# kangxiongbin/HyLight

Hardware: AMD Instinct MI355X
Metric: long-read all-vs-all overlaps/sec (higher is better)
Workload: dtype u8/int32

## Files before the change

### hylight_amd/csrc/filter_stage.hip

```cpp
#include "filter_stage.h"

#include <memory>

#include <algorithm>

#include "dev_prims.h"
#include "dev_search.h"
#include "wave_ops.h"

namespace hlmi {

namespace {

constexpr int WINDOW = 1000;
constexpr int QUERY_CAP = 60;
constexpr int WG = 256;

__device__ __forceinline__ uint64_t pair_key(uint32_t a, uint32_t b) {
    return a <= b ? ((uint64_t)a << 32 | b) : ((uint64_t)b << 32 | a);
}

__device__ __forceinline__ bool is_internal(const PafRec &r, int min_o) {
    int64_t ql = r.qlen, qs = r.qs, qe = r.qe, tl = r.tlen, ts = r.ts, te = r.te;
    if (r.flags & PF_REV) {
// ... 262 lines not shown
        size_t j = i;
        while (j > b && row_less(recs[x], recs[grows[j - 1]], ops)) { grows[j] = grows[j - 1]; --j; }
        grows[j] = x;
    }
    bool taken = false;
    for (size_t i = b; i < e; ++i) {
        const PafRec &r = recs[grows[i]];
        bool s1 = false;
        if (r.qid != r.tid) {
            if (long_mode) {
                if (!(r.flags & PF_STAR) && !taken) { s1 = true; taken = true; }
            } else {
                s1 = true;
            }
        }
        sel[i] = s1;
    }
}

constexpr uint32_t NO_PAIR = 0xffffffffu;
__device__ __forceinline__ uint32_t wave_incl_sum_u32(uint32_t v, int lane) {
    (void)lane;
    return wave_prefix_sum_incl_dpp(v);
}

__global__ __launch_bounds__(WG) void snp_count_kernel(const PafRec *recs, const uint32_t *ops, const uint32_t *grows,
                                                        const uint8_t *sel, size_t n, int long_mode, uint32_t *n_ev,
                                                        uint32_t *n_iv, uint32_t *maxv) {
    const int lane = threadIdx.x & 63;
    const size_t wave = (blockIdx.x * (size_t)blockDim.x + threadIdx.x) >> 6;
    const size_t n_waves = ((size_t)gridDim.x * blockDim.x) >> 6;
    uint32_t max_id = 0, max_len = 0;
    for (size_t i = wave; i < n; i += n_waves) {
        uint32_t ne = 0, ni = 0;
        if (sel[i]) {
            const PafRec &r = recs[grows[i]];
            max_id = max(max_id, max(r.qid, r.tid));
            max_len = max(max_len, max(r.qlen, r.tlen));
            const uint32_t *o = ops + r.cig_off;
            for (uint32_t k0 = 0; k0 < r.cig_n; k0 += 64)
                ne += (uint32_t)__popcll(__ballot(k0 + lane < r.cig_n && (o[k0 + lane] & 15u) == OP_X));
            if (long_mode) ne *= 2;
            ni = (r.ts < r.te ? 1u : 0u) + ((long_mode && r.qs < r.qe) ? 1u : 0u);
        }
        if (lane == 0) { n_ev[i] = ne; n_iv[i] = ni; }
    }
    if (lane == 0) {
        if (max_id > __hip_atomic_load(&maxv[0], __ATOMIC_RELAXED, __HIP_MEMORY_SCOPE_AGENT)) atomicMax(&maxv[0], max_id);
        if (max_len > __hip_atomic_load(&maxv[1], __ATOMIC_RELAXED, __HIP_MEMORY_SCOPE_AGENT)) atomicMax(&maxv[1], max_len);
    }
}

__global__ __launch_bounds__(WG) void snp_fill_kernel(const PafRec *recs, const uint32_t *ops, const uint32_t *grows,
                                                       const uint8_t *sel, size_t n, int long_mode, const uint32_t *ev_off,
                                                       const uint32_t *iv_off, const uint32_t *row_pair, int hb, int lb,
                                                       uint64_t *ev_ck, uint32_t *ev_pair,
                                                       uint64_t *iv_sck, uint64_t *iv_eck) {
    auto ck = [&](uint32_t chunk, uint32_t id, uint32_t pos) { return ((uint64_t)chunk << hb | id) << lb | pos; };
    const int lane = threadIdx.x & 63;
    const size_t wave = (blockIdx.x * (size_t)blockDim.x + threadIdx.x) >> 6;
    const size_t n_waves = ((size_t)gridDim.x * blockDim.x) >> 6;
    for (size_t i = wave; i < n; i += n_waves) {
        if (!sel[i]) continue;
        const PafRec r = recs[grows[i]];
        if (lane == 0) {
            uint32_t w = iv_off[i];
            if (r.ts < r.te) { iv_sck[w] = ck(r.chunk, r.tid, r.ts); iv_eck[w] = ck(r.chunk, r.tid, r.te); ++w; }
            if (long_mode && r.qs < r.qe) { iv_sck[w] = ck(r.chunk, r.qid, r.qs); iv_eck[w] = ck(r.chunk, r.qid, r.qe); }
        }
        const uint32_t pg = row_pair[i];
        const bool rev = r.flags & PF_REV;
        uint32_t p1 = rev ? r.qlen - r.qe : r.qs;
        uint32_t p2 = r.ts;
        uint32_t e = ev_off[i];
        const uint32_t *o = ops + r.cig_off;
        for (uint32_t k0 = 0; k0 < r.cig_n; k0 += 64) {
            uint32_t len = 0, code = 0;
            if (k0 + lane < r.cig_n) { const uint32_t op = o[k0 + lane]; len = op >> 4; code = op & 15u; }
            const bool isx = code == OP_X;
            const uint32_t d1 = (code == OP_EQ || code == OP_I || isx) ? len : 0u;
            const uint32_t d2 = (code == OP_EQ || code == OP_D || isx) ? len : 0u;
            const uint32_t s1 = wave_incl_sum_u32(d1, lane), s2 = wave_incl_sum_u32(d2, lane);
            const unsigned long long xm = __ballot(isx);
            if (isx) {
                const uint32_t q1 = p1 + s1, q2 = p2 + s2;
                uint32_t at = e + (uint32_t)__popcll(xm & ((1ull << lane) - 1ull)) * (long_mode ? 2u : 1u);
                if (long_mode) {
                    const uint32_t qp = rev ? r.qlen - q1 + 1 : q1;
                    ev_ck[at] = ck(r.chunk, r.qid, qp); ev_pair[at] = pg; ++at;
                }
                ev_ck[at] = ck(r.chunk, r.tid, q2); ev_pair[at] = pg;
            }
            p1 += (uint32_t)__shfl((int)s1, 63, 64);
            p2 += (uint32_t)__shfl((int)s2, 63, 64);
            e += (uint32_t)__popcll(xm) * (long_mode ? 2u : 1u);
        }
    }
}

__global__ void snp_support_kernel(const uint64_t *ev_ck, const uint32_t *kseg_start, size_t n_kseg, size_t n_ev,
                                   const uint64_t *ivs_ck, const uint64_t *ive_ck, size_t n_iv, int lb, int mc,
                                   uint8_t *ev_supported) {
    size_t s = blockIdx.x * (size_t)blockDim.x + threadIdx.x;
    if (s >= n_kseg) return;
    size_t b = kseg_start[s], e = (s + 1 < n_kseg) ? kseg_start[s + 1] : n_ev;
    int64_t v = (int64_t)(e - b);
    if (v < mc) return;
    const uint64_t key = ev_ck[b];
    const uint64_t read0 = key >> lb << lb;
    const size_t a = lower_bound_u64(ivs_ck, n_iv, read0);
    const uint64_t next_read = read0 + (1ull << lb);
    size_t span = n_iv - a < 4096 ? n_iv - a : 4096;
    if (span == 4096 && ivs_ck[a + span - 1] < next_read) span = n_iv - a;
    const size_t b_ = a + lower_bound_u64(ivs_ck + a, span, next_read);
    const int64_t n_start_lt = (int64_t)lower_bound_u64(ivs_ck + a, b_ - a, key);
    const int64_t n_end_le = (int64_t)lower_bound_u64(ive_ck + a, b_ - a, key + 1);
    int64_t con = n_start_lt - n_end_le;
    if (con - v < mc) return;
    for (size_t i = b; i < e; ++i) ev_supported[i] = 1;
}

__global__ void snp_pair_count_kernel(const uint32_t *ev_pair_sorted, const uint8_t *ev_supported, size_t n_ev,
                                      uint32_t *pair_mut) {
    size_t i = blockIdx.x * (size_t)blockDim.x + threadIdx.x;
    if (i < n_ev && ev_supported[i]) {
        const uint32_t pg = ev_pair_sorted[i];
        if (pg != NO_PAIR) atomicAdd(&pair_mut[pg], 1u);
    }
}

constexpr int PILE_TILE = 15360;
constexpr int PILE_WG_HEAVY = 1024;
constexpr int PILE_LIGHT_ROWS = 16;
constexpr int PILE_EV_SLOTS = 4096;
constexpr uint32_t PILE_MAX_ROWS = 60000;

__global__ void pile_entries_kernel(const PafRec *recs, const uint32_t *grows, const uint8_t *sel, size_t m, int long_mode,
                                    uint64_t *key, uint32_t *val) {
    size_t i = blockIdx.x * (size_t)blockDim.x + threadIdx.x;
    if (i >= m) return;
    uint64_t kt = ~0ull, kq = ~0ull;
    if (sel[i]) {
        const PafRec &r = recs[grows[i]];
        kt = (uint64_t)r.chunk << 32 | r.tid;
        if (long_mode) kq = (uint64_t)r.chunk << 32 | r.qid;
    }
    key[2 * i] = kt; val[2 * i] = (uint32_t)(i << 1);
    key[2 * i + 1] = kq; val[2 * i + 1] = (uint32_t)(i << 1 | 1u);
}
__global__ void pile_entry_rows_kernel(const uint32_t *ent_val, const uint32_t *grows, size_t n, uint32_t *ent_rec) {
    size_t k = blockIdx.x * (size_t)blockDim.x + threadIdx.x;
    if (k < n) ent_rec[k] = grows[ent_val[k] >> 1];
}
__global__ void add_one_u8_kernel(const uint8_t *in, uint8_t *out, size_t n) {
    size_t i = blockIdx.x * (size_t)blockDim.x + threadIdx.x;
    if (i < n) out[i] = in[i] + 1;
}
__global__ void pile_seg_size_kernel(const uint32_t *seg_start, size_t n_seg, size_t n_ent, uint32_t *max_rows) {
    size_t s = blockIdx.x * (size_t)blockDim.x + threadIdx.x;
    if (s >= n_seg) return;
    const uint32_t n = (uint32_t)((s + 1 < n_seg ? seg_start[s + 1] : n_ent) - seg_start[s]);
    if (n > __hip_atomic_load(max_rows, __ATOMIC_RELAXED, __HIP_MEMORY_SCOPE_AGENT)) atomicMax(max_rows, n);
}

template <typename CT> __device__ __forceinline__ void lds_inc(uint32_t *a, uint32_t idx) {
    constexpr uint32_t per = 4 / sizeof(CT);
    atomicAdd(&a[idx / per], 1u << (8 * sizeof(CT) * (idx % per)));
}
template <typename CT> __device__ __forceinline__ uint32_t lds_get(const uint32_t *a, uint32_t idx) { return ((const CT *)a)[idx]; }

__global__ void pile_seg_class_kernel(const uint32_t *seg_start, size_t n_seg, size_t n_ent, int mc, uint8_t *cls) {
    size_t s = blockIdx.x * (size_t)blockDim.x + threadIdx.x;
    if (s >= n_seg) return;
    const uint32_t n = (uint32_t)((s + 1 < n_seg ? seg_start[s + 1] : n_ent) - seg_start[s]);
    cls[s] = (long long)n < 2ll * mc ? 0 : (n <= (uint32_t)PILE_LIGHT_ROWS ? 1 : 2);
}
__global__ __launch_bounds__(WG) void pile_tiny_events_kernel(const PafRec *recs, const uint32_t *ops, const uint32_t *grows,
                                                               const uint32_t *ent_val, const uint32_t *seg_start, const uint32_t *list,
                                                               size_t n_list, size_t n_seg, size_t n_ent, unsigned long long *n_events) {
    const int lane = threadIdx.x & 63;
    const size_t w = (blockIdx.x * (size_t)blockDim.x + threadIdx.x) >> 6;
    if (w >= n_list) return;
    const size_t seg = list[w];
    const size_t b = seg_start[seg], e = seg + 1 < n_seg ? seg_start[seg + 1] : n_ent;
    unsigned long long ev = 0;
    for (size_t k = b; k < e; ++k) {
        const PafRec &r = recs[grows[ent_val[k] >> 1]];
        const uint32_t *o = ops + r.cig_off;
        for (uint32_t k0 = 0; k0 < r.cig_n; k0 += 64)
            ev += (unsigned long long)__popcll(__ballot(k0 + lane < r.cig_n && (o[k0 + lane] & 15u) == OP_X));
    }
    if (lane == 0 && ev) atomicAdd(&n_events[w & (PILE_EV_SLOTS - 1)], ev);
}

template <int PILE_WG, typename CT>
__global__ __launch_bounds__(PILE_WG) __attribute__((amdgpu_waves_per_eu(8, 8))) void snp_pileup_kernel(const PafRec *recs, const uint32_t *ops, const uint32_t *ent_rec,
                                                              const uint32_t *row_pair, const uint64_t *ent_key, const uint32_t *ent_val,
                                                              const uint32_t *seg_start, const uint32_t *list, size_t n_seg, size_t n_ent,
                                                              int long_mode, int mc, uint32_t *pair_mut, unsigned long long *n_events) {
    constexpr uint32_t PER = 4 / sizeof(CT);
    __shared__ uint32_t sA[PILE_TILE / PER], sB[PILE_TILE / PER];
    __shared__ uint32_t s_part[2][PILE_WG / 64];
    const int tid = threadIdx.x, lane = tid & 63, wave = tid >> 6;
    const size_t seg = list[blockIdx.x];
    const size_t b = seg_start[seg], e = seg + 1 < n_seg ? seg_start[seg + 1] : n_ent;
    __shared__ uint32_t s_len;
    if (tid == 0) s_len = 0;
    __syncthreads();
    {
        uint32_t l = 0;
        for (size_t k = b + (size_t)tid; k < e; k += PILE_WG) {
            const uint32_t v = ent_val[k];
            const PafRec &r = recs[ent_rec[k]];
            l = max(l, (v & 1u) ? r.qlen : r.tlen);
        }
        if (l) atomicMax(&s_len, l);
    }
    __syncthreads();
    const uint32_t read_len = s_len;
    auto walk = [&](const PafRec &r, bool qside, auto &&f) {
        const bool rev = r.flags & PF_REV;
        uint32_t p = qside ? (rev ? r.qlen - r.qe : r.qs) : r.ts;
        const uint32_t skip = qside ? OP_D : OP_I;
        const uint32_t *o = ops + r.cig_off;
        for (uint32_t k0 = 0; k0 < r.cig_n; k0 += 256) {
            uint32_t opv[4];
#pragma unroll
            for (int u = 0; u < 4; ++u) { const uint32_t idx = k0 + 64u * u + lane; opv[u] = idx < r.cig_n ? o[idx] : skip; }
#pragma unroll
            for (int u = 0; u < 4; ++u) {
                if (k0 + 64u * u >= r.cig_n) break;
                const uint32_t len = opv[u] >> 4, code = opv[u] & 15u;
                const bool isx = code == OP_X;
                const uint32_t sc = wave_prefix_sum_incl_dpp(code == skip ? 0u : len);
                const uint32_t after = p + sc;
                f(qside && rev ? r.qlen - after + 1 : after, isx);
                p += (uint32_t)__builtin_amdgcn_readlane((int)sc, 63);
            }
        }
    };
    unsigned long long ev = 0;
    for (uint32_t t0 = 0; t0 < read_len + 2; t0 += PILE_TILE) {
        const uint32_t n_pos = min((uint32_t)PILE_TILE, read_len + 2 - t0), n_words = (n_pos + PER - 1) / PER;
        for (uint32_t w = tid; w < n_words; w += PILE_WG) { sA[w] = 0; sB[w] = 0; }
        __syncthreads();
        for (size_t k = b + (size_t)tid; k < e; k += PILE_WG) {
            const uint32_t v = ent_val[k];
            const PafRec &r = recs[ent_rec[k]];
            const uint32_t s0 = (v & 1u) ? r.qs : r.ts, e0 = (v & 1u) ? r.qe : r.te;
            if (s0 < e0) {
                const uint32_t ia = max(s0 + 1, t0) - t0, ib = max(e0, t0) - t0;
                if (ia < n_pos) lds_inc<CT>(sA, ia);
                if (ib < n_pos) lds_inc<CT>(sB, ib);
            }
        }
        __syncthreads();
        {
            const uint32_t per = (n_pos + PILE_WG - 1) / PILE_WG, lo = min(n_pos, (uint32_t)tid * per), hi = min(n_pos, lo + per);
            uint32_t ta = 0, tb = 0;
            for (uint32_t i = lo; i < hi; ++i) { ta += lds_get<CT>(sA, i); tb += lds_get<CT>(sB, i); }
            const uint32_t ia = wave_prefix_sum_incl_dpp(ta), ib = wave_prefix_sum_incl_dpp(tb);
            if (lane == 63) { s_part[0][wave] = ia; s_part[1][wave] = ib; }
            __syncthreads();
            uint32_t oa = ia - ta, ob = ib - tb;
            for (int w = 0; w < wave; ++w) { oa += s_part[0][w]; ob += s_part[1][w]; }
            CT *ca = (CT *)sA, *cb = (CT *)sB;
            for (uint32_t i = lo; i < hi; ++i) {
                oa += ca[i]; ob += cb[i];
                ca[i] = (CT)(oa - ob);
                cb[i] = 0;
            }
        }
        __syncthreads();
        {
            size_t k = b + (size_t)wave;
            uint32_t v = 0;
            PafRec r{};
            if (k < e) { v = ent_val[k]; r = recs[ent_rec[k]]; }
            while (k < e) {
                const size_t kn = k + PILE_WG / 64;
                uint32_t vn = 0;
                PafRec rn{};
                if (kn < e) { vn = ent_val[kn]; rn = recs[ent_rec[kn]]; }
                walk(r, (v & 1u) != 0, [&](uint32_t pos, bool isx) {
                    if (isx && pos >= t0 && pos - t0 < n_pos) lds_inc<CT>(sB, pos - t0);
                    if (t0 == 0) ev += (unsigned long long)__popcll(__ballot(isx));
                });
                k = kn; v = vn; r = rn;
            }
        }
        __syncthreads();
        {
            auto next_live = [&](size_t k) {
                while (k < e && row_pair[ent_val[k] >> 1] == NO_PAIR) k += PILE_WG / 64;
                return k;
            };
            size_t k = next_live(b + (size_t)wave);
            uint32_t v = 0;
            PafRec r{};
            if (k < e) { v = ent_val[k]; r = recs[ent_rec[k]]; }
            while (k < e) {
                const size_t kn = next_live(k + PILE_WG / 64);
                uint32_t vn = 0;
                PafRec rn{};
                if (kn < e) { vn = ent_val[kn]; rn = recs[ent_rec[kn]]; }
                uint32_t hits = 0;
                walk(r, (v & 1u) != 0, [&](uint32_t pos, bool isx) {
                    if (isx && pos >= t0 && pos - t0 < n_pos) {
                        const int cnt = (int)lds_get<CT>(sB, pos - t0), cov = (int)lds_get<CT>(sA, pos - t0);
                        if (cnt >= mc && cov - cnt >= mc) ++hits;
                    }
                });
                hits = wave_incl_sum_u32(hits, lane);
                if (lane == 63 && hits) atomicAdd(&pair_mut[row_pair[v >> 1]], hits);
                k = kn; v = vn; r = rn;
            }
        }
        __syncthreads();
    }
    if (lane == 0 && ev) atomicAdd(&n_events[(blockIdx.x * 16u + (uint32_t)wave) & (PILE_EV_SLOTS - 1)], ev);
}

constexpr int PILE_LIGHT_WG = 512, PILE_LIGHT_IT = 6;
__global__ __launch_bounds__(PILE_LIGHT_WG) void snp_pileup_light_kernel(const PafRec *recs, const uint32_t *ops, const uint32_t *ent_rec,
                                                                          const uint32_t *row_pair, const uint32_t *ent_val,
                                                                          const uint32_t *seg_start, const uint32_t *list, size_t n_seg,
                                                                          size_t n_ent, int mc, uint32_t *pair_mut,
                                                                          unsigned long long *n_events) {
    __shared__ uint32_t sV[PILE_TILE / 4];
    __shared__ uint32_t s_is[PILE_LIGHT_ROWS], s_ie[PILE_LIGHT_ROWS], s_len;
    __shared__ uint32_t s_ev[PILE_LIGHT_ROWS * 64 * PILE_LIGHT_IT], s_nev, s_hits[PILE_LIGHT_ROWS], s_pair[PILE_LIGHT_ROWS];
    const int tid = threadIdx.x, lane = tid & 63, wave = tid >> 6;
    const size_t seg = list[blockIdx.x];
    const size_t b = seg_start[seg], e = seg + 1 < n_seg ? seg_start[seg + 1] : n_ent;
    const int n_rows = (int)(e - b);
    if (tid == 0) s_len = 0;
    if (tid < PILE_LIGHT_ROWS) s_pair[tid] = NO_PAIR;
    __syncthreads();
    uint32_t pos[2][PILE_LIGHT_IT];
    uint32_t xm[2] = {0, 0}, pg[2] = {NO_PAIR, NO_PAIR};
    bool spill[2] = {false, false};
    PafRec rr[2];
    bool side[2] = {false, false};
    unsigned long long ev = 0;
#pragma unroll
    for (int sl = 0; sl < 2; ++sl) {
        const int k = wave + 8 * sl;
        if (k >= n_rows) continue;
        const uint32_t v = ent_val[b + k];
        const PafRec r = recs[ent_rec[b + k]];
        rr[sl] = r; side[sl] = (v & 1u) != 0;
        pg[sl] = row_pair[v >> 1];
        const bool qside = side[sl], rev = r.flags & PF_REV;
        if (lane == 0) {
            const uint32_t s0 = qside ? r.qs : r.ts, e0 = qside ? r.qe : r.te;
            s_is[k] = s0 < e0 ? s0 : 0; s_ie[k] = s0 < e0 ? e0 : 0;
            s_pair[k] = pg[sl];
            atomicMax(&s_len, qside ? r.qlen : r.tlen);
        }
        spill[sl] = r.cig_n > 64u * PILE_LIGHT_IT;
        uint32_t p = qside ? (rev ? r.qlen - r.qe : r.qs) : r.ts;
        const uint32_t skip = qside ? OP_D : OP_I;
        const uint32_t *o = ops + r.cig_off;
        uint32_t opv[PILE_LIGHT_IT];
#pragma unroll
        for (int u = 0; u < PILE_LIGHT_IT; ++u) { const uint32_t idx = 64u * u + lane; opv[u] = idx < r.cig_n ? o[idx] : skip; }
#pragma unroll
        for (int u = 0; u < PILE_LIGHT_IT; ++u) {
            const uint32_t len = opv[u] >> 4, code = opv[u] & 15u;
            const uint32_t sc = wave_prefix_sum_incl_dpp(code == skip ? 0u : len);
            const uint32_t after = p + sc;
            pos[sl][u] = qside && rev ? r.qlen - after + 1 : after;
            if (code == OP_X) xm[sl] |= 1u << u;
            p += (uint32_t)__builtin_amdgcn_readlane((int)sc, 63);
        }
        for (uint32_t k0 = 0; k0 < r.cig_n; k0 += 64)
            ev += (unsigned long long)__popcll(__ballot(k0 + lane < r.cig_n && (k0 < 64u * PILE_LIGHT_IT ? ((xm[sl] >> (k0 >> 6)) & 1u) != 0
                                                                                 : (o[k0 + lane] & 15u) == OP_X)));
    }
    __syncthreads();
    const uint32_t read_len = s_len;
    auto tail = [&](int sl, auto &&f) {
        const PafRec &r = rr[sl];
        const bool qside = side[sl], rev = r.flags & PF_REV;
        const uint32_t skip = qside ? OP_D : OP_I;
        const uint32_t *o = ops + r.cig_off;
        uint32_t p = qside ? (rev ? r.qlen - r.qe : r.qs) : r.ts;
        for (uint32_t k0 = 0; k0 < r.cig_n; k0 += 64) {
            uint32_t len = 0, code = skip;
            if (k0 + lane < r.cig_n) { const uint32_t op = o[k0 + lane]; len = op >> 4; code = op & 15u; }
            const uint32_t sc = wave_prefix_sum_incl_dpp(code == skip ? 0u : len);
            const uint32_t after = p + sc;
            if (k0 >= 64u * PILE_LIGHT_IT) f(qside && rev ? r.qlen - after + 1 : after, code == OP_X);
            p += (uint32_t)__builtin_amdgcn_readlane((int)sc, 63);
        }
    };
    for (uint32_t t0 = 0; t0 < read_len + 2; t0 += PILE_TILE) {
        const uint32_t n_pos = min((uint32_t)PILE_TILE, read_len + 2 - t0);
        for (uint32_t w = tid; w < (n_pos + 3) / 4; w += PILE_LIGHT_WG) sV[w] = 0;
        if (tid < PILE_LIGHT_ROWS) s_hits[tid] = 0;
        if (tid == 0) s_nev = 0;
        __syncthreads();
#pragma unroll
        for (int sl = 0; sl < 2; ++sl) {
            if (wave + 8 * sl >= n_rows) continue;
#pragma unroll
            for (int u = 0; u < PILE_LIGHT_IT; ++u) {
                const bool in = ((xm[sl] >> u) & 1u) && pos[sl][u] >= t0 && pos[sl][u] - t0 < n_pos;
                if (in) lds_inc<uint8_t>(sV, pos[sl][u] - t0);
                if (pg[sl] != NO_PAIR) {
                    const unsigned long long m = __ballot(in);
                    if (m) {
                        uint32_t at = 0;
                        if (lane == 0) at = atomicAdd(&s_nev, (uint32_t)__popcll(m));
                        at = (uint32_t)__builtin_amdgcn_readfirstlane((int)at);
                        if (in) s_ev[at + (uint32_t)__popcll(m & ((1ull << lane) - 1ull))] = (pos[sl][u] - t0) | (uint32_t)(wave + 8 * sl) << 16;
                    }
                }
            }
            if (spill[sl]) tail(sl, [&](uint32_t q, bool isx) { if (isx && q >= t0 && q - t0 < n_pos) lds_inc<uint8_t>(sV, q - t0); });
        }
        __syncthreads();
        auto supported = [&](uint32_t q) {
            const int cnt = (int)lds_get<uint8_t>(sV, q - t0);
            if (cnt < mc) return false;
            int cov = 0;
            for (int i = 0; i < n_rows; ++i) cov += (s_is[i] < q && q < s_ie[i]) ? 1 : 0;
            return cov - cnt >= mc;
        };
        {
            const uint32_t n_ev = s_nev;
            for (uint32_t i = tid; i < n_ev; i += PILE_LIGHT_WG) {
                const uint32_t w = s_ev[i];
                if (supported(t0 + (w & 0xffffu))) atomicAdd(&s_hits[w >> 16], 1u);
            }
        }
#pragma unroll
        for (int sl = 0; sl < 2; ++sl) {
            if (wave + 8 * sl >= n_rows || pg[sl] == NO_PAIR || !spill[sl]) continue;
            uint32_t hits = 0;
            tail(sl, [&](uint32_t q, bool isx) { if (isx && q >= t0 && q - t0 < n_pos && supported(q)) ++hits; });
            hits = wave_prefix_sum_incl_dpp(hits);
            if (lane == 63 && hits) atomicAdd(&s_hits[wave + 8 * sl], hits);
        }
        __syncthreads();
        if (tid < PILE_LIGHT_ROWS && s_hits[tid]) atomicAdd(&pair_mut[s_pair[tid]], s_hits[tid]);
        __syncthreads();
    }
    if (lane == 0 && ev) atomicAdd(&n_events[(blockIdx.x * 16u + (uint32_t)wave) & (PILE_EV_SLOTS - 1)], ev);
}

__global__ void pair_live_kernel(const PafRec *recs, const uint32_t *grows, const uint32_t *seg_start, size_t n_seg,
                                 size_t n_rows, int len_over, int min_o, uint32_t *row_pair) {
    size_t s = blockIdx.x * (size_t)blockDim.x + threadIdx.x;
    if (s >= n_seg) return;
    size_t b = seg_start[s], e = (s + 1 < n_seg) ? seg_start[s + 1] : n_rows;
    bool any = false;
    for (size_t i = b; i < e && !any; ++i) {
        const PafRec &r = recs[grows[i]];
        any = r.qid != r.tid && (int64_t)r.nmatch >= (int64_t)len_over && !is_internal(r, min_o);
    }
    for (size_t i = b; i < e; ++i) row_pair[i] = any ? (uint32_t)s : 0xffffffffu;
}

__global__ void pass2_kernel(const PafRec *recs, const uint32_t *ops, const uint32_t *grows,
                             const uint32_t *seg_start, size_t n_seg, size_t n_rows, const uint32_t *pair_mut,
                             int long_mode, int len_over, double thre, int min_o, uint8_t *keep, uint32_t *xdig) {
    size_t s = blockIdx.x * (size_t)blockDim.x + threadIdx.x;
    if (s >= n_seg) return;
    size_t b = seg_start[s], e = (s + 1 < n_seg) ? seg_start[s + 1] : n_rows;
    const uint32_t mut = pair_mut[s];
    bool done = false;
    for (size_t i = b; i < e; ++i) {
        keep[i] = 0;
        if (done) continue;
        const PafRec &r = recs[grows[i]];
        if (mut > 0) {
            if (!long_mode) continue;
            if ((double)mut / (double)r.nmatch > thre) continue;
        }
        if (r.qid == r.tid) continue;
        if ((int64_t)r.nmatch < (int64_t)len_over) continue;
        if (is_internal(r, min_o)) continue;
        done = true;
        keep[i] = 1;
        uint32_t sum = 0;
        const uint32_t *o = ops + r.cig_off;
        for (uint32_t k = 0; k < r.cig_n; ++k)
            if ((o[k] & 15u) == OP_X) sum += (o[k] >> 4) % 10u;
        xdig[i] = sum;
    }
}

std::vector<uint64_t> make_windows(const std::vector<uint64_t> &chunk_row_start, std::vector<uint32_t> &len) {
    std::vector<uint64_t> start;
    for (size_t c = 0; c + 1 < chunk_row_start.size(); ++c)
        for (uint64_t p = chunk_row_start[c]; p < chunk_row_start[c + 1]; p += WINDOW) {
            start.push_back(p);
            len.push_back((uint32_t)std::min<uint64_t>(WINDOW, chunk_row_start[c + 1] - p));
        }
    return start;
}

}

namespace {
__global__ void chunk_ops_kernel(const PafRec *recs, size_t n, unsigned long long *ops_of_chunk) {
    size_t i = blockIdx.x * (size_t)blockDim.x + threadIdx.x;
    const bool live = i < n;
    const uint32_t c = live ? recs[i].chunk : 0xffffffffu;
    unsigned long long v = live ? recs[i].cig_n : 0;
    const uint32_t c0 = (uint32_t)__shfl((int)c, 0, 64);
    if (__all(!live || c == c0)) {
#pragma unroll
        for (int o = 32; o > 0; o >>= 1) v += __shfl_xor(v, o, 64);
        if ((threadIdx.x & 63) == 0 && v) atomicAdd(&ops_of_chunk[c0], v);
    } else if (live && v) {
        atomicAdd(&ops_of_chunk[c], v);
    }
}
}

std::vector<uint64_t> ops_per_chunk(const PafRec *d_recs, size_t n, uint32_t n_chunk_ids) {
    DBuf<unsigned long long> acc(n_chunk_ids ? n_chunk_ids : 1);
    acc.zero();
    if (n) hipLaunchKernelGGL(chunk_ops_kernel, grid1(n), dim3(WG), 0, stream(), d_recs, n, acc.p);
    HIP_CHECK(hipGetLastError());
    std::vector<unsigned long long> h = acc.download(n_chunk_ids);
    return std::vector<uint64_t>(h.begin(), h.end());
}

std::vector<PafRec> download_rows(const PafRec *d_recs, const std::vector<uint32_t> &idx) {
    std::vector<PafRec> out;
    if (idx.empty()) return out;
    DBuf<uint32_t> d_idx;
    d_idx.upload(idx);
    DBuf<PafRec> tmp(idx.size());
    hipLaunchKernelGGL(gather_rec_kernel, grid1(idx.size()), dim3(WG), 0, stream(), d_recs, d_idx.p, tmp.p, idx.size());
    HIP_CHECK(hipGetLastError());
    return tmp.download(idx.size());
}

void window_filter_device(const PafRec *d_recs, size_t n, const std::vector<uint64_t> &chunk_row_start, int variant,
                          int min_len, double min_iden, int min_o, uint8_t *d_keep) {
    if (!n) return;
    std::vector<uint32_t> wlen;
    std::vector<uint64_t> wstart = make_windows(chunk_row_start, wlen);
    DBuf<uint64_t> d_ws;
    DBuf<uint32_t> d_wl;
    d_ws.upload(wstart);
    d_wl.upload(wlen);
    if (variant == 4)
        hipLaunchKernelGGL(window_filter_kernel<4>, dim3((unsigned)wstart.size()), dim3(WG), 0, stream(), d_recs, d_ws.p,
                           d_wl.p, min_len, min_iden, min_o, d_keep);
    else if (variant == 3)
        hipLaunchKernelGGL(window_filter_kernel<3>, dim3((unsigned)wstart.size()), dim3(WG), 0, stream(), d_recs, d_ws.p,
                           d_wl.p, min_len, min_iden, min_o, d_keep);
    else
        fail(HLMI_EINVAL, "window filter variant must be 3 or 4");
    HIP_CHECK(hipGetLastError());
    sync();
}

void ovlp_inline_device(const PafRec *d_recs, size_t n, int min_len, double min_iden, int o, double r, uint8_t *d_keep,
                        uint32_t *d_first_of) {
    if (!n) return;
    std::vector<uint32_t> wlen;
    std::vector<uint64_t> wstart = make_windows({0, (uint64_t)n}, wlen);
    DBuf<uint64_t> d_ws;
    DBuf<uint32_t> d_wl;
    d_ws.upload(wstart);
    d_wl.upload(wlen);
    hipLaunchKernelGGL(ovlp_inline_kernel, dim3((unsigned)wstart.size()), dim3(WG), 0, stream(), d_recs, d_ws.p, d_wl.p, min_len,
                       min_iden, o, r, d_keep, d_first_of);
    HIP_CHECK(hipGetLastError());
    sync();
}

void filter_stage_device(const PafRec *d_recs, size_t n, const uint32_t *d_ops,
                         const std::vector<uint64_t> &chunk_row_start, const FilterCfg &cfg, FilterOut &out) {
    out = FilterOut();
    if (!n) return;
    const uint32_t n_chunks = std::max<uint32_t>((uint32_t)(chunk_row_start.size() - 1), cfg.chunk_id_bound);
    const int lm = cfg.long_mode ? 1 : 0;

    std::unique_ptr<HostTimer> ht(new HostTimer("filter_v4_select"));
    DBuf<uint8_t> keep1(n);
    { KTimer kt("filter_v4");
    window_filter_device(d_recs, n, chunk_row_start, 4, cfg.v4_min_len, cfg.v4_min_iden, cfg.v4_min_o, keep1.p);
    }
    DBuf<uint32_t> rows(n);
    const size_t m = select_flagged_indices(keep1.p, rows.p, n);
    out.n_after_v4 = m;
    if (!m) return;

    ht.reset(); ht.reset(new HostTimer("filter_pair_groups"));
    DBuf<uint32_t> rchunk(m);
    DBuf<uint64_t> rkey(m);
    hipLaunchKernelGGL(pair_keys_kernel, grid1(m), dim3(WG), 0, stream(), d_recs, rows.p, m, rchunk.p, rkey.p);
    SortedCK g;
    sort_chunk_key(rchunk.p, rkey.p, m, n_chunks, g);
    DBuf<uint32_t> grows(m);
    hipLaunchKernelGGL(gather_u32_kernel, grid1(m), dim3(WG), 0, stream(), rows.p, g.perm.p, grows.p, m);
    DBuf<uint8_t> head(m);
    hipLaunchKernelGGL(head_flags_kernel, grid1(m), dim3(WG), 0, stream(), g.chunk.p, g.key.p, head.p, m);
    DBuf<uint32_t> pseg_start(m);
    const size_t n_pseg = select_flagged_indices(head.p, pseg_start.p, m);
    out.n_pairs = n_pseg;
    DBuf<uint8_t> sel(m);
    hipLaunchKernelGGL(pair_order_select_kernel, grid1(n_pseg), dim3(WG), 0, stream(), d_recs, d_ops, grows.p, pseg_start.p,
                       n_pseg, m, lm, sel.p);

    ht.reset(); ht.reset(new HostTimer("filter_events"));
    DBuf<uint32_t> pair_mut(n_pseg);
    pair_mut.zero();
    bool piled = false;
    if (!hook("HLMI_SNP_SORT")) {
        DBuf<uint64_t> ekey(2 * m);
        DBuf<uint32_t> eval(2 * m);
        hipLaunchKernelGGL(pile_entries_kernel, grid1(m), dim3(WG), 0, stream(), d_recs, grows.p, sel.p, m, lm, ekey.p, eval.p);
        sort_pairs_u64_u32(ekey, eval, 2 * m, 0, 32 + bits_for(n_chunks > 1 ? n_chunks - 1 : 1));
        DBuf<uint32_t> eseg(2 * m);
        size_t n_eseg = select_run_heads_u64(ekey.p, 2 * m, 0, eseg.p);
        size_t n_ent = 2 * m;
        if (n_eseg && download_one(ekey.p + (2 * m - 1)) == ~0ull) { --n_eseg; n_ent = download_one(eseg.p + n_eseg); }
        DBuf<uint32_t> max_rows(1);
        max_rows.zero();
        if (n_eseg) hipLaunchKernelGGL(pile_seg_size_kernel, grid1(n_eseg), dim3(WG), 0, stream(), eseg.p, n_eseg, n_ent, max_rows.p);
        if (!n_eseg || download_one(max_rows.p) <= PILE_MAX_ROWS) {
            DBuf<uint32_t> row_pair(m);
            DBuf<unsigned long long> n_ev_d(PILE_EV_SLOTS);
            n_ev_d.zero();
            hipLaunchKernelGGL(pair_live_kernel, grid1(n_pseg), dim3(WG), 0, stream(), d_recs, grows.p, pseg_start.p, n_pseg, m,
                               cfg.len_over, cfg.min_o, row_pair.p);
            if (n_eseg) {
                DBuf<uint32_t> erec(n_ent);
                hipLaunchKernelGGL(pile_entry_rows_kernel, grid1(n_ent), dim3(WG), 0, stream(), eval.p, grows.p, n_ent, erec.p);
                DBuf<uint8_t> cls(n_eseg);
                hipLaunchKernelGGL(pile_seg_class_kernel, grid1(n_eseg), dim3(WG), 0, stream(), eseg.p, n_eseg, n_ent, cfg.mc, cls.p);
                DBuf<uint32_t> l0(n_eseg), l1(n_eseg), l2(n_eseg), l3(1), cnt4(4);
                DBuf<uint8_t> cls1(n_eseg);
                hipLaunchKernelGGL(add_one_u8_kernel, grid1(n_eseg), dim3(WG), 0, stream(), cls.p, cls1.p, n_eseg);
                select_classes4_async(cls1.p, n_eseg, l0.p, l1.p, l2.p, l3.p, cnt4.p);
                const std::vector<uint32_t> nc = cnt4.download(4);
                if (nc[0]) hipLaunchKernelGGL(pile_tiny_events_kernel, dim3(cdiv(nc[0], (size_t)(WG / 64))), dim3(WG), 0, stream(), d_recs,
                                              d_ops, grows.p, eval.p, eseg.p, l0.p, (size_t)nc[0], n_eseg, n_ent, n_ev_d.p);
                if (nc[1]) {
                    KTimer kt("filter_pileup_light");
                    hipLaunchKernelGGL(snp_pileup_light_kernel, dim3(nc[1]), dim3(PILE_LIGHT_WG), 0, stream(), d_recs, d_ops, erec.p,
                                       row_pair.p, eval.p, eseg.p, l1.p, n_eseg, n_ent, cfg.mc, pair_mut.p, n_ev_d.p);
                }
                if (nc[2]) {
                    KTimer kt("filter_pileup_heavy");
                    hipLaunchKernelGGL((snp_pileup_kernel<PILE_WG_HEAVY, uint16_t>), dim3(nc[2]), dim3(PILE_WG_HEAVY), 0, stream(), d_recs, d_ops, erec.p,
                                       row_pair.p, ekey.p, eval.p, eseg.p, l2.p, n_eseg, n_ent, lm, cfg.mc, pair_mut.p, n_ev_d.p);
                }
            }
            HIP_CHECK(hipGetLastError());
            {
                const std::vector<unsigned long long> evs = n_ev_d.download(PILE_EV_SLOTS);
                unsigned long long tot = 0;
                for (unsigned long long v : evs) tot += v;
                out.n_events = (size_t)tot;
            }
            piled = true;
        }
    }
    if (!piled) {
    DBuf<uint32_t> n_ev(m), n_iv(m), ev_off(m), iv_off(m);
    const dim3 rows_grid((unsigned)std::min<size_t>(cdiv(m ? m : 1, WG / 64), 65536));
    DBuf<uint32_t> maxv(2);
    maxv.zero();
    hipLaunchKernelGGL(snp_count_kernel, rows_grid, dim3(WG), 0, stream(), d_recs, d_ops, grows.p, sel.p, m, lm, n_ev.p,
                       n_iv.p, maxv.p);
    exclusive_scan_u32(n_ev.p, ev_off.p, m);
    exclusive_scan_u32(n_iv.p, iv_off.p, m);
    const size_t E = (size_t)download_one(ev_off.p + (m - 1)) + download_one(n_ev.p + (m - 1));
    const size_t I = (size_t)download_one(iv_off.p + (m - 1)) + download_one(n_iv.p + (m - 1));
    out.n_events = E;
    if (E) {
        const std::vector<uint32_t> mx = maxv.download(2);
        const int cb = bits_for(n_chunks > 1 ? n_chunks - 1 : 1), hb = bits_for(mx[0] ? mx[0] : 1), lb = bits_for((uint64_t)mx[1] + 1);
        if (cb + hb + lb > 64) fail(HLMI_EINVAL, "SNP pile-up key needs %d bits (chunks %d, reads %d, positions %d)", cb + hb + lb, cb, hb, lb);
        DBuf<uint32_t> ev_pair(E);
        DBuf<uint64_t> ev_ck(E), iv_sck(I ? I : 1), iv_eck(I ? I : 1);
    { KTimer kt("filter_event_fill");
        DBuf<uint32_t> row_pair(m);
        hipLaunchKernelGGL(pair_live_kernel, grid1(n_pseg), dim3(WG), 0, stream(), d_recs, grows.p, pseg_start.p, n_pseg, m,
                           cfg.len_over, cfg.min_o, row_pair.p);
        hipLaunchKernelGGL(snp_fill_kernel, rows_grid, dim3(WG), 0, stream(), d_recs, d_ops, grows.p, sel.p, m, lm,
                           ev_off.p, iv_off.p, row_pair.p, hb, lb, ev_ck.p, ev_pair.p, iv_sck.p, iv_eck.p);
    }
    { KTimer kt("filter_event_sort");
        sort_pairs_u64_u32(ev_ck, ev_pair, E, 0, cb + hb + lb);
        sort_keys_u64(iv_sck, I, 0, cb + hb + lb);
        sort_keys_u64(iv_eck, I, 0, cb + hb + lb);
    }
        DBuf<uint32_t> kseg_start(E);
        const size_t n_kseg = select_run_heads_u64(ev_ck.p, E, 0, kseg_start.p);

        DBuf<uint8_t> ev_sup(E);
        ev_sup.zero();
    { KTimer kt("filter_support");
        hipLaunchKernelGGL(snp_support_kernel, grid1(n_kseg), dim3(WG), 0, stream(), ev_ck.p, kseg_start.p, n_kseg, E,
                           iv_sck.p, iv_eck.p, I, lb, cfg.mc, ev_sup.p);
    }
    { KTimer kt("filter_pair_count");
        hipLaunchKernelGGL(snp_pair_count_kernel, grid1(E), dim3(WG), 0, stream(), ev_pair.p, ev_sup.p, E, pair_mut.p);
    }
        HIP_CHECK(hipGetLastError());
        sync();
    }

    }

    ht.reset(); ht.reset(new HostTimer("filter_pass2_order"));
    DBuf<uint8_t> keep2(m);
    DBuf<uint32_t> xdig(m);
    xdig.zero();
    hipLaunchKernelGGL(pass2_kernel, grid1(n_pseg), dim3(WG), 0, stream(), d_recs, d_ops, grows.p, pseg_start.p, n_pseg,
                       m, pair_mut.p, lm, cfg.len_over, cfg.thre, cfg.min_o, keep2.p, xdig.p);
    HIP_CHECK(hipGetLastError());
    DBuf<uint32_t> kidx(m);
    const size_t nk = select_flagged_indices(keep2.p, kidx.p, m);
    if (!nk) return;
    DBuf<uint32_t> krows(nk), kx(nk);
    hipLaunchKernelGGL(gather_u32_kernel, grid1(nk), dim3(WG), 0, stream(), grows.p, kidx.p, krows.p, nk);
    hipLaunchKernelGGL(gather_u32_kernel, grid1(nk), dim3(WG), 0, stream(), xdig.p, kidx.p, kx.p, nk);
    std::vector<uint32_t> hrows = krows.download(nk), hx = kx.download(nk);
    if (!cfg.reference_order) {
        out.rows.swap(hrows);
        out.x_digit_sum.swap(hx);
        return;
    }
    std::vector<PafRec> hrecs(nk);
    {
        DBuf<PafRec> tmp(nk);
        hipLaunchKernelGGL(gather_rec_kernel, grid1(nk), dim3(WG), 0, stream(), d_recs, krows.p, tmp.p, nk);
        hrecs = tmp.download(nk);
    }
    std::vector<uint32_t> ord(nk);
    for (size_t i = 0; i < nk; ++i) ord[i] = (uint32_t)i;
    std::sort(ord.begin(), ord.end(), [&](uint32_t a, uint32_t b) {
        const PafRec &x = hrecs[a], &y = hrecs[b];
        if (x.chunk != y.chunk) return x.chunk < y.chunk;
        if (x.tlen != y.tlen) return x.tlen < y.tlen;
        if (x.ts != y.ts) return x.ts < y.ts;
        if (x.te != y.te) return x.te < y.te;
        return x.tie < y.tie;
    });
    out.rows.resize(nk);
    out.x_digit_sum.resize(nk);
    for (size_t i = 0; i < nk; ++i) {
        out.rows[i] = hrows[ord[i]];
        out.x_digit_sum[i] = hx[ord[i]];
    }
}

}
```

### hylight_amd/csrc/runtime.cpp

```cpp
#include <mutex>

#include "common.h"
#include <sched.h>

#include <iterator>

namespace hlmi {

namespace {
thread_local std::string g_last_error;
bool g_ready = false;
int g_device = 0;
int g_threads = 0;
std::map<std::string, double> g_stats;
std::mutex g_mu;
std::mutex g_stat_mu;

struct KRec { std::string name; hipEvent_t a, b; hipStream_t s; };
struct Lane {
    hipStream_t stream = nullptr, side = nullptr;
    std::vector<KRec> krecs;
    void *pinned = nullptr;
};
Lane g_lanes[MAX_LANES];
// ... 13 lines not shown
    }
    return g_threads;
}

void *pinned_scratch() {
    void *&p = lane().pinned;
    if (!p) HIP_CHECK(hipHostMalloc(&p, PINNED_SCRATCH_BYTES, hipHostMallocDefault));
    return p;
}

void init_device(int device, int threads) {
    std::lock_guard<std::mutex> lk(g_mu);
    int n = 0;
    hipError_t e = hipGetDeviceCount(&n);
    if (e != hipSuccess || n <= 0)
        fail(HLMI_ENODEV, "no HIP device available (%s); libhylight_mi has no CPU fallback",
             e != hipSuccess ? hipGetErrorString(e) : "device count is 0");
    if (device >= n) fail(HLMI_EINVAL, "device %d out of range (have %d)", device, n);
    if (device >= 0) HIP_CHECK(hipSetDevice(device));
    HIP_CHECK(hipGetDevice(&g_device));
    if (!g_lanes[0].stream) HIP_CHECK(hipStreamCreateWithFlags(&g_lanes[0].stream, hipStreamNonBlocking));
    if (threads > 0) g_threads = threads;
    g_ready = true;
}

void shutdown_device() {
    std::lock_guard<std::mutex> lk(g_mu);
    dev_pool_trim();
    for (Lane &l : g_lanes) {
        for (hipStream_t *st : {&l.side, &l.stream}) {
            if (!*st) continue;
            (void)hipStreamSynchronize(*st);
            (void)hipStreamDestroy(*st);
            *st = nullptr;
        }
    }
    g_ready = false;
}

void require_device() {
    if (!g_ready) init_device(-1, 0);
}

hipStream_t stream() { return lane().stream; }
hipStream_t side_stream_if_created() { return lane().side; }
hipStream_t side_stream() {
    hipStream_t &g_side = lane().side;
    if (!g_side) {
        int least = 0, greatest = 0;
        if (hipDeviceGetStreamPriorityRange(&least, &greatest) != hipSuccess) { (void)hipGetLastError(); greatest = 0; }
        HIP_CHECK(hipStreamCreateWithPriority(&g_side, hipStreamNonBlocking, greatest));
    }
    return g_side;
}

static void lane_drain() {
    Lane &l = lane();
    if (l.stream) (void)hipStreamSynchronize(l.stream);
    if (l.side) (void)hipStreamSynchronize(l.side);
}

KTimer::KTimer(const char *name, hipStream_t on) {
    KRec r;
    r.name = name;
    r.s = on ? on : lane().stream;
    HIP_CHECK(hipEventCreate(&r.a));
    HIP_CHECK(hipEventCreate(&r.b));
    HIP_CHECK(hipEventRecord(r.a, r.s));
    slot = lane().krecs.size();
    lane().krecs.push_back(r);
}
KTimer::~KTimer() { (void)hipEventRecord(lane().krecs[slot].b, lane().krecs[slot].s); }

void ktimer_flush() {
    auto &krecs = lane().krecs;
    if (krecs.empty()) return;
    lane_drain();
    std::lock_guard<std::mutex> lk(g_stat_mu);
    for (auto &r : krecs) {
        float ms = 0;
        if (hipEventElapsedTime(&ms, r.a, r.b) == hipSuccess) {
            g_stats["kernel_ms." + r.name] += ms;
            g_stats["kernel_launches." + r.name] += 1;
        }
        (void)hipEventDestroy(r.a);
        (void)hipEventDestroy(r.b);
    }
    krecs.clear();
}

size_t ktimer_mark() { return lane().krecs.size(); }
void ktimer_rollback(size_t mark) {
    auto &krecs = lane().krecs;
    if (mark >= krecs.size()) return;
    lane_drain();
    for (size_t i = mark; i < krecs.size(); ++i) { (void)hipEventDestroy(krecs[i].a); (void)hipEventDestroy(krecs[i].b); }
    krecs.resize(mark);
}

void ktimer_discard() {
    auto &krecs = lane().krecs;
    if (krecs.empty()) return;
    lane_drain();
    for (auto &r : krecs) { (void)hipEventDestroy(r.a); (void)hipEventDestroy(r.b); }
    krecs.clear();
}

int lane_count() {
    int n = 2;
    if (const char *e = hook("HLMI_LANES")) n = atoi(e);
    return std::max(1, std::min(n, MAX_LANES));
}
LaneScope::LaneScope(int id) : prev(t_lane) {
    if (id < 0 || id >= MAX_LANES) fail(HLMI_EINVAL, "lane %d out of range", id);
    t_lane = id;
    HIP_CHECK(hipSetDevice(g_device));
    if (!lane().stream) HIP_CHECK(hipStreamCreateWithFlags(&lane().stream, hipStreamNonBlocking));
}
LaneScope::~LaneScope() {
    lane_drain();
    try { ktimer_flush(); } catch (...) {}
    t_lane = prev;
}

namespace {
const char *const HOOK_NAMES[] = {
    "HLMI_ALIGN_SPAN_TASKS",
    "HLMI_ANCHOR_BATCH_M",
    "HLMI_ANCHOR_PAIRS",
    "HLMI_ANCHOR_SPLIT",
    "HLMI_ASM_STAGE_CAP",
    "HLMI_ASM_WAVE",
    "HLMI_CHAIN_DP16_CHECK",
    "HLMI_CHAIN_NO_DP16",
    "HLMI_CHAIN_NO_SMALL",
    "HLMI_SEED_GROUP", "HLMI_TEXT_GPU", "HLMI_TEXT_HOST", "HLMI_GRAPH_WINDOW_MB", "HLMI_LANES", "HLMI_SET_ASIDE_CUTS", "HLMI_SEED_NO_GUESS",
    "HLMI_CHAIN_PROF",
    "HLMI_CHAIN_UNPACKED",
    "HLMI_CLASSIFY_BYTES",
    "HLMI_GROUP_HIST",
    "HLMI_HOST_TIMERS",
    "HLMI_LONG_SIDE_STREAM",
    "HLMI_NARROW_LONG_UNPACKED",
    "HLMI_NARROW_UNPACKED",
    "HLMI_NO_EXT_CERT",
    "HLMI_POLISH_ROWS_GRID",
    "HLMI_NO_GAP1_CERT",
    "HLMI_NO_GAP2_CERT",
    "HLMI_NO_ONE_PIECE_CERT",
    "HLMI_NO_RANK_WORD",
    "HLMI_NO_SHIFT_CERT",
    "HLMI_NO_STUB",
    "HLMI_NO_SUFFIX_TRIM",
    "HLMI_QCAP_MIN",
    "HLMI_RUN_BUF_CAP",
    "HLMI_SKETCH_PART_MBASES",
    "HLMI_SNP_SORT",
    "HLMI_STUB_FULL_ROWS",
    "HLMI_SUBRUN_MAX_MANCHORS",
    "HLMI_SUBRUN_MAX_OUT_MB",
    "HLMI_SUBRUN_MBASES"};
std::unordered_map<std::string, std::string> g_hooks;
}
void hooks_refresh() {
    g_hooks.clear();
    for (const char *n : HOOK_NAMES)
        if (const char *v = getenv(n)) g_hooks[n] = v;
}
const char *hook(const char *name) {
    bool known = false;
    for (const char *n : HOOK_NAMES) known = known || strcmp(n, name) == 0;
    if (!known) fail(HLMI_EINVAL, "hook %s is not in the table of runtime.cpp", name);
    auto it = g_hooks.find(name);
    return it == g_hooks.end() ? nullptr : it->second.c_str();
}

namespace {
struct CachedBlock { void *p; int lane; };
std::multimap<size_t, CachedBlock> g_free_blocks;
std::mutex g_pool_mu;
std::unordered_map<void *, size_t> g_block_size;
size_t g_pooled_bytes = 0;
size_t g_owned_bytes = 0;
size_t g_peak_in_use = 0;
constexpr size_t POOL_CAP = 160ull << 30;
constexpr size_t GRAN = 2ull << 20;
}

static size_t size_class(size_t bytes) {
    size_t want = (bytes + GRAN - 1) / GRAN * GRAN;
    if (want > (64ull << 20)) {
        size_t p2 = 1;
        while ((p2 << 1) <= want) p2 <<= 1;
        const size_t step = p2 >> 3;
        want = (want + step - 1) / step * step;
    }
    return want;
}

static void pool_trim_locked() {
    (void)hipDeviceSynchronize();
    for (auto &kv : g_free_blocks) {
        (void)hipFree(kv.second.p);
        g_owned_bytes -= kv.first;
        g_block_size.erase(kv.second.p);
    }
    g_free_blocks.clear();
    g_pooled_bytes = 0;
}

void *dev_alloc(size_t bytes) {
    const size_t want = size_class(bytes);
    std::lock_guard<std::mutex> lk(g_pool_mu);
    auto it = g_free_blocks.lower_bound(want);
    {
        int looked = 0;
        for (auto own = it; own != g_free_blocks.end() && own->first <= want + want / 2 && looked < 16; ++own, ++looked)
            if (own->second.lane == t_lane) { it = own; break; }
    }
    if (it != g_free_blocks.end() && it->first <= want + want / 2) {
        void *p = it->second.p;
        const int from = it->second.lane;
        if (from != t_lane && g_lanes[from].stream && lane().stream) {
            hipEvent_t ev;
            HIP_CHECK(hipEventCreateWithFlags(&ev, hipEventDisableTiming));
            HIP_CHECK(hipEventRecord(ev, g_lanes[from].stream));
            HIP_CHECK(hipStreamWaitEvent(lane().stream, ev, 0));
            if (lane().side) HIP_CHECK(hipStreamWaitEvent(lane().side, ev, 0));
            HIP_CHECK(hipEventDestroy(ev));
        }
        g_pooled_bytes -= it->first;
        g_free_blocks.erase(it);
        g_peak_in_use = std::max(g_peak_in_use, g_owned_bytes - g_pooled_bytes);
        return p;
    }
    if (!g_free_blocks.empty()) {
        size_t free_b = 0, total_b = 0;
        if (hipMemGetInfo(&free_b, &total_b) == hipSuccess) {
            bool drained = false;
            while (free_b < want + (1ull << 30) && !g_free_blocks.empty()) {
                if (!drained) { (void)hipDeviceSynchronize(); drained = true; }
                auto big = std::prev(g_free_blocks.end());
                (void)hipFree(big->second.p);
                g_block_size.erase(big->second.p);
                g_pooled_bytes -= big->first;
                g_owned_bytes -= big->first;
                free_b += big->first;
                g_free_blocks.erase(big);
            }
        } else (void)hipGetLastError();
    }
    void *p = nullptr;
    hipError_t e = hipMalloc(&p, want);
    if (e != hipSuccess) {
        (void)hipGetLastError();
        pool_trim_locked();
        e = hipMalloc(&p, want);
        if (e != hipSuccess) (void)hipGetLastError();
    }
    if (e != hipSuccess) fail(HLMI_ENOMEM, "hipMalloc of %zu bytes failed: %s", want, hipGetErrorString(e));
    g_block_size[p] = want;
    g_owned_bytes += want;
    g_peak_in_use = std::max(g_peak_in_use, g_owned_bytes - g_pooled_bytes);
    return p;
}

size_t dev_peak_bytes(bool reset) {
    std::lock_guard<std::mutex> lk(g_pool_mu);
    const size_t v = g_peak_in_use;
    if (reset) g_peak_in_use = g_owned_bytes - g_pooled_bytes;
    return v;
}

size_t dev_available_bytes() {
    size_t free_b = 0, total_b = 0;
    if (hipMemGetInfo(&free_b, &total_b) != hipSuccess) { (void)hipGetLastError(); return 0; }
    std::lock_guard<std::mutex> lk(g_pool_mu);
    return free_b + g_pooled_bytes;
}

void dev_free(void *p) {
    std::lock_guard<std::mutex> lk(g_pool_mu);
    auto it = g_block_size.find(p);
    if (it == g_block_size.end()) { (void)hipFree(p); return; }
    if (g_pooled_bytes + it->second > POOL_CAP) {
        (void)hipFree(p);
        g_owned_bytes -= it->second;
        g_block_size.erase(it);
        return;
    }
    g_free_blocks.emplace(it->second, CachedBlock{p, t_lane});
    g_pooled_bytes += it->second;
}

void dev_pool_trim() {
    std::lock_guard<std::mutex> lk(g_pool_mu);
    pool_trim_locked();
}

static double wall_s() {
    timespec ts;
    clock_gettime(CLOCK_MONOTONIC, &ts);
    return (double)ts.tv_sec + 1e-9 * (double)ts.tv_nsec;
}
static bool host_timers_on() {
    const bool on = hook("HLMI_HOST_TIMERS") != nullptr;
// ... 20 lines not shown
```

Before: 3664.

## Skip dead light pileup segments and count events on target side only

Segment classification now checks row liveness and target presence. Light segments with no live pair are downgraded to event-only counting, and segments with no target-side entry are skipped entirely. Event counting is done only for target-side entries, and the total is doubled in long mode instead of walking both sides. The events kernel now batches record loads across lanes, the add-one kernel is removed, and a hook restores the old behaviour. The doubling assumes query-side and target-side X counts are symmetric, which is a correctness risk if that does not hold.

```diff
diff --git a/hylight_amd/csrc/filter_stage.hip b/hylight_amd/csrc/filter_stage.hip
--- a/hylight_amd/csrc/filter_stage.hip
+++ b/hylight_amd/csrc/filter_stage.hip
@@ -438,10 +438,6 @@
     size_t k = blockIdx.x * (size_t)blockDim.x + threadIdx.x;
     if (k < n) ent_rec[k] = grows[ent_val[k] >> 1];
 }
-__global__ void add_one_u8_kernel(const uint8_t *in, uint8_t *out, size_t n) {
-    size_t i = blockIdx.x * (size_t)blockDim.x + threadIdx.x;
-    if (i < n) out[i] = in[i] + 1;
-}
 __global__ void pile_seg_size_kernel(const uint32_t *seg_start, size_t n_seg, size_t n_ent, uint32_t *max_rows) {
     size_t s = blockIdx.x * (size_t)blockDim.x + threadIdx.x;
     if (s >= n_seg) return;
@@ -455,26 +451,63 @@
 }
 template <typename CT> __device__ __forceinline__ uint32_t lds_get(const uint32_t *a, uint32_t idx) { return ((const CT *)a)[idx]; }
 
-__global__ void pile_seg_class_kernel(const uint32_t *seg_start, size_t n_seg, size_t n_ent, int mc, uint8_t *cls) {
-    size_t s = blockIdx.x * (size_t)blockDim.x + threadIdx.x;
-    if (s >= n_seg) return;
-    const uint32_t n = (uint32_t)((s + 1 < n_seg ? seg_start[s + 1] : n_ent) - seg_start[s]);
-    cls[s] = (long long)n < 2ll * mc ? 0 : (n <= (uint32_t)PILE_LIGHT_ROWS ? 1 : 2);
-}
-__global__ __launch_bounds__(WG) void pile_tiny_events_kernel(const PafRec *recs, const uint32_t *ops, const uint32_t *grows,
-                                                               const uint32_t *ent_val, const uint32_t *seg_start, const uint32_t *list,
-                                                               size_t n_list, size_t n_seg, size_t n_ent, unsigned long long *n_events) {
+enum : uint8_t { PILE_CLS_NONE = 0, PILE_CLS_EVENTS = 1, PILE_CLS_LIGHT = 2, PILE_CLS_HEAVY = 3 };
+__global__ __launch_bounds__(WG) void pile_seg_class_kernel(const uint32_t *seg_start, size_t n_seg, size_t n_ent,
+                                                             const uint32_t *ent_val, const uint32_t *row_pair, int mc, int pile_all,
+                                                             uint8_t *cls, uint32_t *n_light) {
+    const size_t s = blockIdx.x * (size_t)blockDim.x + threadIdx.x;
+    bool light = false, dead = false;
+    if (s < n_seg) {
+        const size_t b = seg_start[s], e = s + 1 < n_seg ? seg_start[s + 1] : n_ent;
+        const size_t n = e - b;
+        uint8_t c = PILE_CLS_HEAVY;
+        if ((long long)n < 2ll * mc || n <= (size_t)PILE_LIGHT_ROWS) {
+            light = !((long long)n < 2ll * mc);
+            bool live = false, target = false;
+            for (size_t k = b; k < e; ++k) {
+                const uint32_t v = ent_val[k];
+                target = target || !(v & 1u);
+                live = live || (light && row_pair[v >> 1] != NO_PAIR);
+            }
+            dead = light && !live;
+            c = light && (live || pile_all) ? PILE_CLS_LIGHT : (target || pile_all) ? PILE_CLS_EVENTS : PILE_CLS_NONE;
+        }
+        cls[s] = c;
+    }
+    const uint32_t nl = (uint32_t)__popcll(__ballot(light)), nd = (uint32_t)__popcll(__ballot(dead));
+    if ((threadIdx.x & 63) == 0) {
+        if (nl) atomicAdd(&n_light[0], nl);
+        if (nd) atomicAdd(&n_light[1], nd);
+    }
+}
+__global__ __launch_bounds__(WG) void pile_events_kernel(const PafRec *recs, const uint32_t *ops, const uint32_t *grows,
+                                                          const uint32_t *ent_val, const uint32_t *seg_start, const uint32_t *list,
+                                                          size_t n_list, size_t n_seg, size_t n_ent, int ev_both,
+                                                          unsigned long long *n_events) {
     const int lane = threadIdx.x & 63;
     const size_t w = (blockIdx.x * (size_t)blockDim.x + threadIdx.x) >> 6;
     if (w >= n_list) return;
     const size_t seg = list[w];
     const size_t b = seg_start[seg], e = seg + 1 < n_seg ? seg_start[seg + 1] : n_ent;
     unsigned long long ev = 0;
-    for (size_t k = b; k < e; ++k) {
-        const PafRec &r = recs[grows[ent_val[k] >> 1]];
-        const uint32_t *o = ops + r.cig_off;
-        for (uint32_t k0 = 0; k0 < r.cig_n; k0 += 64)
-            ev += (unsigned long long)__popcll(__ballot(k0 + lane < r.cig_n && (o[k0 + lane] & 15u) == OP_X));
+    for (size_t k0 = b; k0 < e; k0 += 64) {
+        const int n_here = e - k0 < 64 ? (int)(e - k0) : 64;
+        unsigned long long off = 0;
+        uint32_t cn = 0;
+        if (lane < n_here) {
+            const uint32_t v = ent_val[k0 + (size_t)lane];
+            if (ev_both || !(v & 1u)) {
+                const PafRec &r = recs[grows[v >> 1]];
+                off = r.cig_off; cn = r.cig_n;
+            }
+        }
+        for (int j = 0; j < n_here; ++j) {
+            const uint32_t n_ops = (uint32_t)__shfl((int)cn, j, 64);
+            if (!n_ops) continue;
+            const uint32_t *o = ops + (unsigned long long)__shfl((long long)off, j, 64);
+            for (uint32_t i0 = 0; i0 < n_ops; i0 += 64)
+                ev += (unsigned long long)__popcll(__ballot(i0 + lane < n_ops && (o[i0 + lane] & 15u) == OP_X));
+        }
     }
     if (lane == 0 && ev) atomicAdd(&n_events[w & (PILE_EV_SLOTS - 1)], ev);
 }
@@ -483,7 +516,8 @@
 __global__ __launch_bounds__(PILE_WG) __attribute__((amdgpu_waves_per_eu(8, 8))) void snp_pileup_kernel(const PafRec *recs, const uint32_t *ops, const uint32_t *ent_rec,
                                                               const uint32_t *row_pair, const uint64_t *ent_key, const uint32_t *ent_val,
                                                               const uint32_t *seg_start, const uint32_t *list, size_t n_seg, size_t n_ent,
-                                                              int long_mode, int mc, uint32_t *pair_mut, unsigned long long *n_events) {
+                                                              int long_mode, int mc, int ev_both, uint32_t *pair_mut,
+                                                              unsigned long long *n_events) {
     constexpr uint32_t PER = 4 / sizeof(CT);
     __shared__ uint32_t sA[PILE_TILE / PER], sB[PILE_TILE / PER];
     __shared__ uint32_t s_part[2][PILE_WG / 64];
@@ -568,9 +602,10 @@
                 uint32_t vn = 0;
                 PafRec rn{};
                 if (kn < e) { vn = ent_val[kn]; rn = recs[ent_rec[kn]]; }
+                const bool count_ev = t0 == 0 && (ev_both || !(v & 1u));
                 walk(r, (v & 1u) != 0, [&](uint32_t pos, bool isx) {
                     if (isx && pos >= t0 && pos - t0 < n_pos) lds_inc<CT>(sB, pos - t0);
-                    if (t0 == 0) ev += (unsigned long long)__popcll(__ballot(isx));
+                    if (count_ev) ev += (unsigned long long)__popcll(__ballot(isx));
                 });
                 k = kn; v = vn; r = rn;
             }
@@ -611,7 +646,7 @@
 __global__ __launch_bounds__(PILE_LIGHT_WG) void snp_pileup_light_kernel(const PafRec *recs, const uint32_t *ops, const uint32_t *ent_rec,
                                                                           const uint32_t *row_pair, const uint32_t *ent_val,
                                                                           const uint32_t *seg_start, const uint32_t *list, size_t n_seg,
-                                                                          size_t n_ent, int mc, uint32_t *pair_mut,
+                                                                          size_t n_ent, int mc, int ev_both, uint32_t *pair_mut,
                                                                           unsigned long long *n_events) {
     __shared__ uint32_t sV[PILE_TILE / 4];
     __shared__ uint32_t s_is[PILE_LIGHT_ROWS], s_ie[PILE_LIGHT_ROWS], s_len;
@@ -660,6 +695,7 @@
             if (code == OP_X) xm[sl] |= 1u << u;
             p += (uint32_t)__builtin_amdgcn_readlane((int)sc, 63);
         }
+        if (!ev_both && qside) continue;
         for (uint32_t k0 = 0; k0 < r.cig_n; k0 += 64)
             ev += (unsigned long long)__popcll(__ballot(k0 + lane < r.cig_n && (k0 < 64u * PILE_LIGHT_IT ? ((xm[sl] >> (k0 >> 6)) & 1u) != 0
                                                                                  : (o[k0 + lane] & 15u) == OP_X)));
@@ -901,6 +937,7 @@
     DBuf<uint32_t> pair_mut(n_pseg);
     pair_mut.zero();
     bool piled = false;
+    const bool pile_all = hook("HLMI_PILE_ALL_SEGMENTS") != nullptr;
     if (!hook("HLMI_SNP_SORT")) {
         DBuf<uint64_t> ekey(2 * m);
         DBuf<uint32_t> eval(2 * m);
@@ -919,27 +956,34 @@
             n_ev_d.zero();
             hipLaunchKernelGGL(pair_live_kernel, grid1(n_pseg), dim3(WG), 0, stream(), d_recs, grows.p, pseg_start.p, n_pseg, m,
                                cfg.len_over, cfg.min_o, row_pair.p);
+            stat_add("pile_light_segments", 0);
+            stat_add("pile_light_segments_dead", 0);
             if (n_eseg) {
                 DBuf<uint32_t> erec(n_ent);
                 hipLaunchKernelGGL(pile_entry_rows_kernel, grid1(n_ent), dim3(WG), 0, stream(), eval.p, grows.p, n_ent, erec.p);
                 DBuf<uint8_t> cls(n_eseg);
-                hipLaunchKernelGGL(pile_seg_class_kernel, grid1(n_eseg), dim3(WG), 0, stream(), eseg.p, n_eseg, n_ent, cfg.mc, cls.p);
-                DBuf<uint32_t> l0(n_eseg), l1(n_eseg), l2(n_eseg), l3(1), cnt4(4);
-                DBuf<uint8_t> cls1(n_eseg);
-                hipLaunchKernelGGL(add_one_u8_kernel, grid1(n_eseg), dim3(WG), 0, stream(), cls.p, cls1.p, n_eseg);
-                select_classes4_async(cls1.p, n_eseg, l0.p, l1.p, l2.p, l3.p, cnt4.p);
-                const std::vector<uint32_t> nc = cnt4.download(4);
-                if (nc[0]) hipLaunchKernelGGL(pile_tiny_events_kernel, dim3(cdiv(nc[0], (size_t)(WG / 64))), dim3(WG), 0, stream(), d_recs,
-                                              d_ops, grows.p, eval.p, eseg.p, l0.p, (size_t)nc[0], n_eseg, n_ent, n_ev_d.p);
+                DBuf<uint32_t> l0(n_eseg), l1(n_eseg), l2(n_eseg), l3(1), cnt(6);
+                cnt.zero();
+                hipLaunchKernelGGL(pile_seg_class_kernel, grid1(n_eseg), dim3(WG), 0, stream(), eseg.p, n_eseg, n_ent, eval.p,
+                                   row_pair.p, cfg.mc, pile_all ? 1 : 0, cls.p, cnt.p + 4);
+                select_classes4_async(cls.p, n_eseg, l0.p, l1.p, l2.p, l3.p, cnt.p);
+                const std::vector<uint32_t> nc = cnt.download(6);
+                stat_add("pile_light_segments", (double)nc[4]);
+                stat_add("pile_light_segments_dead", (double)nc[5]);
+                if (nc[0]) {
+                    KTimer kt("filter_pileup_events");
+                    hipLaunchKernelGGL(pile_events_kernel, dim3(cdiv(nc[0], (size_t)(WG / 64))), dim3(WG), 0, stream(), d_recs, d_ops,
+                                       grows.p, eval.p, eseg.p, l0.p, (size_t)nc[0], n_eseg, n_ent, pile_all ? 1 : 0, n_ev_d.p);
+                }
                 if (nc[1]) {
                     KTimer kt("filter_pileup_light");
                     hipLaunchKernelGGL(snp_pileup_light_kernel, dim3(nc[1]), dim3(PILE_LIGHT_WG), 0, stream(), d_recs, d_ops, erec.p,
-                                       row_pair.p, eval.p, eseg.p, l1.p, n_eseg, n_ent, cfg.mc, pair_mut.p, n_ev_d.p);
+                                       row_pair.p, eval.p, eseg.p, l1.p, n_eseg, n_ent, cfg.mc, pile_all ? 1 : 0, pair_mut.p, n_ev_d.p);
                 }
                 if (nc[2]) {
                     KTimer kt("filter_pileup_heavy");
                     hipLaunchKernelGGL((snp_pileup_kernel<PILE_WG_HEAVY, uint16_t>), dim3(nc[2]), dim3(PILE_WG_HEAVY), 0, stream(), d_recs, d_ops, erec.p,
-                                       row_pair.p, ekey.p, eval.p, eseg.p, l2.p, n_eseg, n_ent, lm, cfg.mc, pair_mut.p, n_ev_d.p);
+                                       row_pair.p, ekey.p, eval.p, eseg.p, l2.p, n_eseg, n_ent, lm, cfg.mc, pile_all ? 1 : 0, pair_mut.p, n_ev_d.p);
                 }
             }
             HIP_CHECK(hipGetLastError());
@@ -947,7 +991,7 @@
                 const std::vector<unsigned long long> evs = n_ev_d.download(PILE_EV_SLOTS);
                 unsigned long long tot = 0;
                 for (unsigned long long v : evs) tot += v;
-                out.n_events = (size_t)tot;
+                out.n_events = (size_t)(lm && !pile_all ? 2 * tot : tot);
             }
             piled = true;
         }
diff --git a/hylight_amd/csrc/runtime.cpp b/hylight_amd/csrc/runtime.cpp
--- a/hylight_amd/csrc/runtime.cpp
+++ b/hylight_amd/csrc/runtime.cpp
@@ -189,6 +189,7 @@
     "HLMI_NO_SHIFT_CERT",
     "HLMI_NO_STUB",
     "HLMI_NO_SUFFIX_TRIM",
+    "HLMI_PILE_ALL_SEGMENTS",
     "HLMI_QCAP_MIN",
     "HLMI_RUN_BUF_CAP",
     "HLMI_SKETCH_PART_MBASES",
```

New measurement: 3631. No clear change (-0.9%).
